# QuanjianSong/UniVST

Measured on AMD Instinct MI355X. Metric: stylized frames/sec, SD-v1.5 16x512x512 @50 DDIM steps, higher is better.
Workload: dtype f16; 1 GPU; sd15_unet_three_branch_pnp_transfer_16x512x512_50ddim; frames=16, branches=3, schedule_steps=53 (wrapping modulo 50), masks=moving disc, blended on steps 0..45, parallelism=single, weights=random-init SD-v1.5 architecture (859M + 201M temporal params), fp16

## Files before the change

### univst_amd/csrc/attention.hip

```cpp
#include <string.h>

#include "common.h"
#include "kernels.h"

namespace {

constexpr int KT = 64;
constexpr float DEFER = 8.f;

typedef __fp16 fh2 __attribute__((ext_vector_type(2)));

__device__ __forceinline__ float max3f(float a, float b, float c) {
    float r;
    asm("v_max3_f32 %0, %1, %2, %3" : "=v"(r) : "v"(a), "v"(b), "v"(c));
    return r;
}

__device__ __forceinline__ void attn_merge_coef(float m1, float l1, float m2, float l2, float& w1, float& w2) {
    const bool has1 = l1 > 0.f, has2 = l2 > 0.f;
    const float m = has1 ? (has2 ? fmaxf(m1, m2) : m1) : m2;
    const float a1 = has1 ? l1 * __builtin_amdgcn_exp2f(m1 - m) : 0.f;
    const float a2 = has2 ? __builtin_amdgcn_exp2f(m2 - m) : 0.f;
    const float den = a1 + l2 * a2;
    const float inv = den > 0.f ? 1.f / den : 0.f;
// ... 323 lines not shown
    for (int qb = 0; qb < QB; ++qb) {
        float l;
        if (ONES) {
            l = __shfl(o[DV16 - 1][qb][0], 32 + l15, 64);
        } else {
            l = lrun[qb];
            l += __shfl_xor(l, 16, 64);
            l += __shfl_xor(l, 32, 64);
        }
        float inv = 1.f / l, w1 = 0.f;
        const int qrow = qblk * 64 * QB + wave * 16 * QB + qb * 16 + l15;
        if (qrow >= p.Nq) continue;
        half_t* op = p.o + ((long)bf * p.Nq + qrow) * p.ldo + h * d;
        if constexpr (TP != 0) {
            const float m2 = CF ? mrun[qb] : mrun[qb] * c;
            const long srow = (((long)bf * p.heads + h) * p.Nq + qrow) * 2;
            if constexpr (TP == 1) {
                if (g == 0) *reinterpret_cast<float2*>(p.state_out + srow) = make_float2(m2, l);
            } else {
                const float2 st = *reinterpret_cast<const float2*>(p.state_in + srow);
                attn_merge_coef(st.x, st.y, m2, l, w1, inv);
            }
        }
#pragma unroll
        for (int dv = 0; dv < DV16; ++dv) {
            const int dc = dv * 16 + g * 4;
            if (dc < d) {
                h4 ov;
                if constexpr (TP == 2) {
                    const h4 o1 = *reinterpret_cast<const h4*>(op + dc);
#pragma unroll
                    for (int r = 0; r < 4; ++r) ov[r] = (half_t)fmaf((float)o1[r], w1, o[dv][qb][r] * inv);
                } else {
#pragma unroll
                    for (int r = 0; r < 4; ++r) ov[r] = (half_t)(o[dv][qb][r] * inv);
                }
                *reinterpret_cast<h4*>(op + dc) = ov;
            }
        }
    }
}

template <int DPAD, int DV16, int QB, bool CF = false, int TP = 0>
__global__ __launch_bounds__(256) void attn_kernel(AttnParams p) {
    attn_body<DPAD, DV16, QB, CF, TP>(p);
}
template <int DPAD, int DV16, int QB, bool CF = false, int TP = 0>
__global__ __launch_bounds__(256, 3) void attn_kernel_occ3(AttnParams p) {
    attn_body<DPAD, DV16, QB, CF, TP>(p);
}

__device__ __attribute__((aligned(256))) half_t uv_attn_zero_page[128];

template <int TAG = 0, int STG = 0, bool K16 = false, int TP = 0>
__global__ __launch_bounds__(256, 2) void attn_pp40_kernel(AttnParams p) {
    constexpr int NW = 4;
    constexpr int D = 40, DV16 = 3, QB = 4, NST = 3;
    constexpr int KSTR = lds_stride_bytes(64 * 2) / 2;
    constexpr int VSTR = lds_stride_bytes(48 * 2) / 2;
    constexpr int KPL = 512, VPL = 576;
    constexpr int KAREA = STG ? 8 * KPL : KT * KSTR;
    constexpr int TILE = STG ? 8 * KPL + 6 * VPL : KT * KSTR + KT * VSTR;
    __shared__ __attribute__((aligned(16))) half_t smem[NST * TILE];

    const int tid = threadIdx.x, lane = tid & 63, wave = tid >> 6;
    const int l15 = lane & 15, g = lane >> 4;
    const int nqb = (p.Nq + 64 * NW - 1) / (64 * NW);
    const int lid = xcd_remap(blockIdx.x, gridDim.x);
    const int qblk = lid % nqb;
    const int h = p.order ? lid / (nqb * p.BF) : (lid / nqb) % p.heads;
    const int bf = p.order ? (lid / nqb) % p.BF : lid / (nqb * p.heads);
    const h8 zero8 = {0, 0, 0, 0, 0, 0, 0, 0};

    const int ntile = (p.Nkv + KT - 1) / KT;
    const int nsrc_eff = p.src_cnt ? p.src_cnt[bf] : p.nsrc;
    const int T = nsrc_eff * ntile;
    if (TP && T == 0) {
        attn_empty_phase<64 * NW>(p, bf, h, qblk, D);
        return;
    }
    float lw_cur = p.src_logw ? p.src_logw[bf * p.nsrc] : 0.f;

    h8 qf[QB][2];
#pragma unroll
    for (int qb = 0; qb < QB; ++qb) {
        const int qrow = qblk * 64 * NW + wave * 16 * QB + qb * 16 + l15;
#pragma unroll
        for (int ks = 0; ks < 2; ++ks) {
            const int dc = ks * 32 + g * 8;
            h8 v = (qrow < p.Nq && dc < D) ? *reinterpret_cast<const h8*>(p.q + ((long)bf * p.Nq + qrow) * p.ldq + h * D + dc) : zero8;
            qf[qb][ks] = v;
        }
        if (!K16 && g == 1) qf[qb][1][2] = (half_t)lw_cur;
        if (K16) {
            h8 v = zero8;
            if (qrow < p.Nq && g < 2) {
                const h4 t = *reinterpret_cast<const h4*>(p.q + ((long)bf * p.Nq + qrow) * p.ldq + h * D + 32 + g * 4);
                v[0] = t[0]; v[1] = t[1]; v[2] = t[2]; v[3] = t[3];
            }
            if (g == 2) v[2] = (half_t)lw_cur;
            qf[qb][1] = v;
        }
    }
    auto set_shift = [&](int qb, float M) -> float {
        const float hi = floorf(M * 0.125f) * 8.f, lo = M - hi;
        const half_t hh = (half_t)(-hi), lh = (half_t)(-lo);
// ... 88 lines not shown
            const int pl = wave_u + NW * j;
            if ((j + 1) * NW <= 2 * DCH || pl < 2 * DCH) {
                const bool isv = pl >= DCH;
                const int c = isv ? pl - DCH : pl;
                const half_t* src = rok ? (isv ? p.v : p.k) + roff + c * 8 : zpage;
                const int dst = stage_half + (isv ? KAREA + c * VPL : c * KPL);
                glds16(src, __builtin_amdgcn_readfirstlane(smem_lds + 2u * (unsigned)dst));
            }
        }
        advance_ld();
    };
    {
        for (int i = tid * 8; i < NST * TILE; i += NW * 64 * 8) *reinterpret_cast<h8*>(&smem[i]) = zero8;
        __syncthreads();
        if (tid < KT) {
#pragma unroll
            for (int st = 0; st < NST; ++st) {
                if (STG) {
                    smem[st * TILE + KAREA + 5 * VPL + tid * 8] = (half_t)1.f;
                    smem[st * TILE + 5 * KPL + tid * 8] = (half_t)1.f;
                    smem[st * TILE + 5 * KPL + tid * 8 + 1] = (half_t)1.f;
                    smem[st * TILE + 5 * KPL + tid * 8 + 2] = (half_t)1.f;
                } else {
                    smem[st * TILE + KT * KSTR + tid * VSTR + D] = (half_t)1.f;
                    smem[st * TILE + tid * KSTR + D] = (half_t)1.f;
                    smem[st * TILE + tid * KSTR + D + 1] = (half_t)1.f;
                    smem[st * TILE + tid * KSTR + D + 2] = (half_t)1.f;
                }
            }
        }
        if (STG) __syncthreads();
    }

    const int kf_off = STG ? g * KPL + l15 * 8 : l15 * KSTR + g * 8;
    const int vf_off = STG ? KAREA + ((l15 & 3) >> 1) * VPL + (g * 4 + (l15 >> 2)) * 8 + (l15 & 1) * 4
                           : KT * KSTR + (g * 4 + (l15 >> 2)) * VSTR + (l15 & 3) * 4;
    auto kfrag_read = [&](const half_t* st, int hh, h8 (&kf)[2][2]) {
#pragma unroll
        for (int kb = 0; kb < 2; ++kb)
#pragma unroll
            for (int ks = 0; ks < 2; ++ks) {
                if (K16 && ks == 1) {
                    const int o16 = STG ? (4 + (g >> 1)) * KPL + l15 * 8 + (g & 1) * 4 + (hh * 32 + kb * 16) * 8
                                        : l15 * KSTR + 32 + g * 4 + (hh * 32 + kb * 16) * KSTR;
                    const h4 t = *reinterpret_cast<const h4*>(&st[o16]);
                    h8 v = zero8;
                    v[0] = t[0]; v[1] = t[1]; v[2] = t[2]; v[3] = t[3];
                    kf[kb][1] = v;
                } else {
                    kf[kb][ks] = *reinterpret_cast<const h8*>(&st[kf_off + (STG ? (hh * 32 + kb * 16) * 8 + ks * 4 * KPL : (hh * 32 + kb * 16) * KSTR + ks * 32)]);
                }
            }
    };
    auto vfrag_read = [&](const half_t* st, int hh, h8 (&vf)[DV16]) {
#pragma unroll
        for (int dv = 0; dv < DV16; ++dv) {
            const half_t* vp = &st[vf_off + (STG ? hh * 32 * 8 + dv * 2 * VPL : hh * 32 * VSTR + dv * 16)];
            fh4 lo = __builtin_amdgcn_ds_read_tr16_b64_v4f16((__attribute__((address_space(3))) fh4*)(vp));
            fh4 hi = __builtin_amdgcn_ds_read_tr16_b64_v4f16((__attribute__((address_space(3))) fh4*)(vp + 16 * (STG ? 8 : VSTR)));
            h8 a;
            a[0] = (half_t)lo[0]; a[1] = (half_t)lo[1]; a[2] = (half_t)lo[2]; a[3] = (half_t)lo[3];
            a[4] = (half_t)hi[0]; a[5] = (half_t)hi[1]; a[6] = (half_t)hi[2]; a[7] = (half_t)hi[3];
            vf[dv] = a;
        }
    };
    auto lo4 = [](const h8& v) { h4 r; r[0] = v[0]; r[1] = v[1]; r[2] = v[2]; r[3] = v[3]; return r; };
    auto qk_a = [&](const h8 (&kf)[2][2], f4 (&sc)[2][QB]) {
        const f4 z = {0.f, 0.f, 0.f, 0.f};
#pragma unroll
        for (int kb = 0; kb < 2; ++kb)
#pragma unroll
            for (int qb = 0; qb < QB; ++qb) sc[kb][qb] = __builtin_amdgcn_mfma_f32_16x16x16f16(lo4(kf[kb][1]), lo4(qf[qb][1]), z, 0, 0, 0);
    };
    auto qk_fence = [&](f4 (&sc)[2][QB]) {
        asm volatile("" : "+v"(qf[0][0]), "+v"(qf[1][0]), "+v"(qf[2][0]), "+v"(qf[3][0])
                     : "v"(sc[0][0]), "v"(sc[0][1]), "v"(sc[0][2]), "v"(sc[0][3]), "v"(sc[1][0]), "v"(sc[1][1]), "v"(sc[1][2]), "v"(sc[1][3]));
    };
    auto qk_b = [&](const h8 (&kf)[2][2], f4 (&sc)[2][QB]) {
#pragma unroll
        for (int kb = 0; kb < 2; ++kb)
#pragma unroll
            for (int qb = 0; qb < QB; ++qb) sc[kb][qb] = __builtin_amdgcn_mfma_f32_16x16x32_f16(kf[kb][0], qf[qb][0], sc[kb][qb], 0, 0, 0);
    };
    auto qk = [&](const h8 (&kf)[2][2], f4 (&sc)[2][QB]) {
        const f4 z = {0.f, 0.f, 0.f, 0.f};
        if (K16) {
            qk_a(kf, sc);
            qk_fence(sc);
            __builtin_amdgcn_sched_barrier(0);
            qk_b(kf, sc);
            return;
        }
#pragma unroll
        for (int kb = 0; kb < 2; ++kb)
#pragma unroll
            for (int qb = 0; qb < QB; ++qb) sc[kb][qb] = __builtin_amdgcn_mfma_f32_16x16x32_f16(kf[kb][0], qf[qb][0], z, 0, 0, 0);
#pragma unroll
        for (int kb = 0; kb < 2; ++kb)
#pragma unroll
            for (int qb = 0; qb < QB; ++qb) sc[kb][qb] = __builtin_amdgcn_mfma_f32_16x16x32_f16(kf[kb][1], qf[qb][1], sc[kb][qb], 0, 0, 0);
    };
    auto exp_part = [&](const f4 (&sc)[2][QB], h8 (&pb)[QB]) {
#pragma unroll
        for (int qb = 0; qb < QB; ++qb) {
            union { fh2 h[4]; h8 v; } u;
#pragma unroll
            for (int kb = 0; kb < 2; ++kb) {
                const float e0 = __builtin_amdgcn_exp2f(sc[kb][qb][0]), e1 = __builtin_amdgcn_exp2f(sc[kb][qb][1]);
                const float e2 = __builtin_amdgcn_exp2f(sc[kb][qb][2]), e3 = __builtin_amdgcn_exp2f(sc[kb][qb][3]);
                u.h[kb * 2] = __builtin_amdgcn_cvt_pkrtz(e0, e1);
                u.h[kb * 2 + 1] = __builtin_amdgcn_cvt_pkrtz(e2, e3);
            }
            pb[qb] = u.v;
        }
    };
    auto exp_half = [&](const f4 (&sc)[2][QB], h8 (&pb)[QB], int half) {
#pragma unroll
        for (int q2 = 0; q2 < 2; ++q2) {
            const int qb = half * 2 + q2;
            union { fh2 h[4]; h8 v; } u;
#pragma unroll
            for (int kb = 0; kb < 2; ++kb) {
                const float e0 = __builtin_amdgcn_exp2f(sc[kb][qb][0]), e1 = __builtin_amdgcn_exp2f(sc[kb][qb][1]);
                const float e2 = __builtin_amdgcn_exp2f(sc[kb][qb][2]), e3 = __builtin_amdgcn_exp2f(sc[kb][qb][3]);
                u.h[kb * 2] = __builtin_amdgcn_cvt_pkrtz(e0, e1);
                u.h[kb * 2 + 1] = __builtin_amdgcn_cvt_pkrtz(e2, e3);
            }
            pb[qb] = u.v;
        }
    };
    auto pv = [&](const h8 (&vf)[DV16], const h8 (&pb)[QB]) {
#pragma unroll
        for (int dv = 0; dv < DV16; ++dv)
#pragma unroll
            for (int qb = 0; qb < QB; ++qb) o[dv][qb] = __builtin_amdgcn_mfma_f32_16x16x32_f16(vf[dv], pb[qb], o[dv][qb], 0, 0, 0);
    };
    auto local_max = [&](const f4 (&sc)[2][QB], float (&mx)[QB]) {
#pragma unroll
        for (int qb = 0; qb < QB; ++qb) {
            float m = max3f(sc[0][qb][0], sc[0][qb][1], sc[0][qb][2]);
            m = max3f(m, sc[0][qb][3], sc[1][qb][0]);
            m = max3f(m, sc[1][qb][1], sc[1][qb][2]);
            mx[qb] = max3f(m, sc[1][qb][3], sc[1][qb][3]);
        }
    };
    auto mask_tail = [&](f4 (&sc)[2][QB], int key0) {
#pragma unroll
        for (int kb = 0; kb < 2; ++kb)
#pragma unroll
            for (int qb = 0; qb < QB; ++qb)
#pragma unroll
                for (int r = 0; r < 4; ++r)
                    if (key0 + kb * 16 + g * 4 + r >= p.Nkv) sc[kb][qb][r] = -INFINITY;
    };
    auto decide = [&](f4 (&sc)[2][QB], const float (&mx)[QB], bool first) {
        if (!first) {
            const float mall = fmaxf(max3f(mx[0], mx[1], mx[2]), mx[3]);
            if (__builtin_amdgcn_ballot_w64(mall > DEFER) == 0) return;
        }
#pragma unroll
        for (int qb = 0; qb < QB; ++qb) {
            if (__builtin_amdgcn_ballot_w64(first || mx[qb] > DEFER) != 0) {
                float m = mx[qb];
                const float o16 = __shfl_xor(m, 16, 64);
                m = max3f(m, o16, o16);
                const float o32 = __shfl_xor(m, 32, 64);
                m = max3f(m, o32, o32);
                float delta = floorf(m * 64.f + 0.5f) * (1.f / 64.f);
                if (!first) delta = fmaxf(delta, 0.f);
                const float mnew = set_shift(qb, mrun[qb] + delta);
                delta = mnew - mrun[qb];
                mrun[qb] = mnew;
                const float alpha = first ? 1.f : __builtin_amdgcn_exp2f(-delta);
#pragma unroll
                for (int kb = 0; kb < 2; ++kb) {
                    sc[kb][qb][0] -= delta; sc[kb][qb][1] -= delta; sc[kb][qb][2] -= delta; sc[kb][qb][3] -= delta;
                }
#pragma unroll
                for (int dv = 0; dv < DV16; ++dv) {
                    o[dv][qb][0] *= alpha; o[dv][qb][1] *= alpha; o[dv][qb][2] *= alpha; o[dv][qb][3] *= alpha;
                }
            }
        }
    };
    auto set_lw = [&](float lw) {
        if (g == (K16 ? 2 : 1)) {
#pragma unroll
            for (int qb = 0; qb < QB; ++qb) qf[qb][1][2] = (half_t)lw;
        }
    };
#define UV_PP_PHASE1()                                                            \
    _Pragma("unroll") for (int i_ = 0; i_ < 16; ++i_) {                           \
        __builtin_amdgcn_sched_group_barrier(0x008, 1, 0);                        \
        if (i_ < 6) __builtin_amdgcn_sched_group_barrier(0x100, 1, 0);            \
        __builtin_amdgcn_sched_group_barrier(0x400, 2, 0);                        \
        __builtin_amdgcn_sched_group_barrier(0x002, 1, 0);                        \
    }
 \
#define UV_PP_PHASE1H(DS)                                                         \
    _Pragma("unroll") for (int i_ = 0; i_ < 8; ++i_) {                            \
        __builtin_amdgcn_sched_group_barrier(0x008, 1, 0);                        \
        if ((DS) && i_ < 6) __builtin_amdgcn_sched_group_barrier(0x100, 1, 0);    \
        __builtin_amdgcn_sched_group_barrier(0x400, 2, 0);                        \
        __builtin_amdgcn_sched_group_barrier(0x002, 1, 0);                        \
    }
#define UV_PP_PHASE2()                                                            \
    _Pragma("unroll") for (int i_ = 0; i_ < 12; ++i_) {                           \
        __builtin_amdgcn_sched_group_barrier(0x008, 1, 0);                        \
        if (i_ < 4) __builtin_amdgcn_sched_group_barrier(0x100, 1, 0);            \
        __builtin_amdgcn_sched_group_barrier(0x002, 2, 0);                        \
    }

#define UV_PP_PIN4(a) asm volatile("" : "+v"(a[0]), "+v"(a[1]), "+v"(a[2]), "+v"(a[3]))
#define UV_PP_PIN2(a, i) asm volatile("" : "+v"(a[i]), "+v"(a[(i) + 1]))

    if (STG) {
        dma_tile(0);
        if (T > 1) dma_tile(TILE);
        asm volatile("s_waitcnt vmcnt(0)" ::: "memory");
    } else {
        load_tile();
        store_tile(smem);
        if (T > 1) {
            load_tile();
            store_tile(smem + TILE);
        }
    }
    __syncthreads();

    f4 scA[2][QB], scB[2][QB];
    h8 kf[2][2], vf[DV16], pb[QB];
    float mx[QB];
    int nx_s = 0, nx_t = (ntile > 1) ? 1 : 0;
    if (ntile == 1) nx_s = 1;
    float lw_nxt = (nx_s != 0 && nx_s < nsrc_eff && p.src_logw) ? p.src_logw[bf * p.nsrc + nx_s] : lw_cur;
    int t0_cur = 0, t0_nxt = nx_t * KT;
    half_t* b_cur = smem;
    half_t* b_nxt = smem + TILE;
    half_t* b_ld = smem + 2 * TILE;

    kfrag_read(b_cur, 0, kf);
    qk(kf, scA);
    if (t0_cur + KT > p.Nkv) mask_tail(scA, t0_cur);
    local_max(scA, mx);
    decide(scA, mx, true);
    kfrag_read(b_cur, 1, kf);

    for (int tt = 0; tt < T; ++tt) {
        const bool has_next = tt + 1 < T;
        if (tt + 2 < T) {
            if (STG) dma_tile((int)(b_ld - smem));
            else load_tile();
        }
        vfrag_read(b_cur, 0, vf);
        if (K16) {
            qk_a(kf, scB);
            exp_half(scA, pb, 0);
            UV_PP_PIN2(pb, 0);
            UV_PP_PHASE1H(1);
            qk_fence(scB);
            __builtin_amdgcn_sched_barrier(0);
            qk_b(kf, scB);
            exp_half(scA, pb, 1);
            UV_PP_PIN2(pb, 2);
            UV_PP_PHASE1H(0);
        } else {
            qk(kf, scB);
            exp_part(scA, pb);
            UV_PP_PIN4(pb);
            UV_PP_PHASE1();
        }
        __builtin_amdgcn_sched_barrier(0);
        if (t0_cur + KT > p.Nkv) mask_tail(scB, t0_cur + 32);
        kfrag_read(b_nxt, 0, kf);
        pv(vf, pb);
        local_max(scB, mx);
        UV_PP_PIN4(mx);
        UV_PP_PHASE2();
        __builtin_amdgcn_sched_barrier(0);
        decide(scB, mx, false);
        if (lw_nxt != lw_cur) set_lw(lw_nxt);
        vfrag_read(b_cur, 1, vf);
        if (K16) {
            qk_a(kf, scA);
            exp_half(scB, pb, 0);
            UV_PP_PIN2(pb, 0);
            UV_PP_PHASE1H(1);
            qk_fence(scA);
            __builtin_amdgcn_sched_barrier(0);
            qk_b(kf, scA);
            exp_half(scB, pb, 1);
            UV_PP_PIN2(pb, 2);
            UV_PP_PHASE1H(0);
        } else {
            qk(kf, scA);
            exp_part(scB, pb);
            UV_PP_PIN4(pb);
            UV_PP_PHASE1();
        }
        __builtin_amdgcn_sched_barrier(0);
        if (has_next && t0_nxt + KT > p.Nkv) mask_tail(scA, t0_nxt);
        kfrag_read(b_nxt, 1, kf);
        pv(vf, pb);
        local_max(scA, mx);
        UV_PP_PIN4(mx);
        UV_PP_PHASE2();
        __builtin_amdgcn_sched_barrier(0);
        if (has_next) decide(scA, mx, false);
        if (!STG && tt + 2 < T) store_tile(b_ld);
        if (STG) asm volatile("s_waitcnt vmcnt(0)" ::: "memory");
        __syncthreads();
        half_t* tb = b_cur; b_cur = b_nxt; b_nxt = b_ld; b_ld = tb;
        t0_cur = t0_nxt;
        lw_cur = lw_nxt;
        if (++nx_t == ntile) {
            nx_t = 0;
            if (++nx_s < nsrc_eff && p.src_logw) lw_nxt = p.src_logw[bf * p.nsrc + nx_s];
        }
        t0_nxt = nx_t * KT;
    }
#undef UV_PP_PHASE1
#undef UV_PP_PHASE1H
#undef UV_PP_PIN2
#undef UV_PP_PIN4
#undef UV_PP_PHASE2

#pragma unroll
    for (int qb = 0; qb < QB; ++qb) {
        const float l = __shfl(o[DV16 - 1][qb][0], 32 + l15, 64);
        float inv = 1.f / l, w1 = 0.f;
        const int qrow = qblk * 64 * NW + wave * 16 * QB + qb * 16 + l15;
        if (qrow >= p.Nq) continue;
        half_t* op = p.o + ((long)bf * p.Nq + qrow) * p.ldo + h * D;
        if constexpr (TP != 0) {
            const float m2 = mrun[qb];
            const long srow = (((long)bf * p.heads + h) * p.Nq + qrow) * 2;
            if constexpr (TP == 1) {
                if (g == 0) *reinterpret_cast<float2*>(p.state_out + srow) = make_float2(m2, l);
            } else {
                const float2 st = *reinterpret_cast<const float2*>(p.state_in + srow);
                attn_merge_coef(st.x, st.y, m2, l, w1, inv);
            }
        }
#pragma unroll
        for (int dv = 0; dv < DV16; ++dv) {
            const int dc = dv * 16 + g * 4;
            if (dc < D) {
                h4 ov;
                if constexpr (TP == 2) {
                    const h4 o1 = *reinterpret_cast<const h4*>(op + dc);
#pragma unroll
                    for (int r = 0; r < 4; ++r) ov[r] = (half_t)fmaf((float)o1[r], w1, o[dv][qb][r] * inv);
                } else {
#pragma unroll
                    for (int r = 0; r < 4; ++r) ov[r] = (half_t)(o[dv][qb][r] * inv);
                }
                *reinterpret_cast<h4*>(op + dc) = ov;
            }
        }
    }
}

template <int TAG = 0, int TP = 0>
__global__ __launch_bounds__(256, 2) void attn_pp64_kernel(AttnParams p) {
    constexpr int D = 64, QB = 4;
    constexpr int NW = 4, DV16 = D / 16, NST = 3;
    constexpr int KS = D / 32;
    constexpr int NDK = D / 8, NPV = D / 8;
    constexpr int RB = NW * 16 * QB;
    constexpr int KPL = 512, VPL = 576;
    constexpr int KAREA = NDK * KPL;
    constexpr int TILE = NDK * KPL + NPV * VPL;
    __shared__ __attribute__((aligned(16))) half_t smem[NST * TILE];

    const int tid = threadIdx.x, lane = tid & 63, wave = tid >> 6;
// ... 43 lines not shown
    const half_t* const zpage = uv_attn_zero_page;
    const unsigned smem_lds = (unsigned)(size_t)((__attribute__((address_space(3))) half_t*)smem);
    auto glds16 = [](const half_t* src, unsigned lds_byte) {
        unsigned keep;
        asm volatile("s_mov_b32 %0, m0\n\ts_mov_b32 m0, %2\n\ts_nop 0\n\tglobal_load_lds_dwordx4 %1, off\n\ts_mov_b32 m0, %0"
                     : "=&s"(keep) : "v"(src), "s"(lds_byte) : "memory");
    };
    const long xk_delta = p.kx ? (long)(p.kx - p.k) : 0, xv_delta = p.kx ? (long)(p.vx - p.v) : 0;
    int ld_s = 0, ld_t = 0;
    long ld_koff, ld_voff, ld_ld;
    int ld_nkv, ld_ntile;
    {
        const long off = (long)__builtin_amdgcn_readfirstlane(p.src_idx[bf * p.nsrc]) * p.Nkv * p.ldkv + h * D;
        ld_koff = off; ld_voff = off; ld_ld = p.ldkv; ld_nkv = p.Nkv; ld_ntile = ntile;
    }
    auto dma_tile = [&](int stage_half) {
        const int t0 = ld_t * KT;
        const bool rok = t0 + lane < ld_nkv;
        const long roff = (long)(t0 + lane) * ld_ld;
        const half_t* const ksrc = p.k + ld_koff + roff;
        const half_t* const vsrc = p.v + ld_voff + roff;
#pragma unroll
        for (int j = 0; j < (NDK + NPV + NW - 1) / NW; ++j) {
            const int pl = wave_u + NW * j;
            if ((j + 1) * NW <= NDK + NPV || pl < NDK + NPV) {
                const bool isv = pl >= NDK;
                const int c = isv ? pl - NDK : pl;
                const half_t* src = rok ? (isv ? vsrc : ksrc) + c * 8 : zpage;
                const int dst = stage_half + (isv ? KAREA + c * VPL : c * KPL);
                glds16(src, __builtin_amdgcn_readfirstlane(smem_lds + 2u * (unsigned)dst));
            }
        }
        if (++ld_t == ld_ntile) {
            ld_t = 0;
            ++ld_s;
            if (ld_s < nsrc_eff) {
                const long off = (long)__builtin_amdgcn_readfirstlane(p.src_idx[bf * p.nsrc + ld_s]) * p.Nkv * p.ldkv + h * D;
                ld_koff = off; ld_voff = off;
            } else if (ld_s < nseg) {
                const long off = (long)__builtin_amdgcn_readfirstlane(p.x_idx[bf]) * p.Nkv_x * p.ldkv_x + h * D;
                ld_koff = off + xk_delta; ld_voff = off + xv_delta; ld_ld = p.ldkv_x; ld_nkv = p.Nkv_x; ld_ntile = ntile_x;
            }
        }
    };

    const int kf_off = g * KPL + l15 * 8;
    const int vf_off = KAREA + ((l15 & 3) >> 1) * VPL + (g * 4 + (l15 >> 2)) * 8 + (l15 & 1) * 4;
    auto kfrag_read = [&](const half_t* st, int hh, h8 (&kf)[2][KS]) {
#pragma unroll
        for (int kb = 0; kb < 2; ++kb)
#pragma unroll
            for (int ks = 0; ks < KS; ++ks) kf[kb][ks] = *reinterpret_cast<const h8*>(&st[kf_off + (hh * 32 + kb * 16) * 8 + ks * 4 * KPL]);
    };
    auto vfrag_read = [&](const half_t* st, int hh, h8 (&vf)[DV16]) {
#pragma unroll
        for (int dv = 0; dv < DV16; ++dv) {
            const half_t* vp = &st[vf_off + hh * 32 * 8 + dv * 2 * VPL];
            fh4 lo = __builtin_amdgcn_ds_read_tr16_b64_v4f16((__attribute__((address_space(3))) fh4*)(vp));
            fh4 hi = __builtin_amdgcn_ds_read_tr16_b64_v4f16((__attribute__((address_space(3))) fh4*)(vp + 16 * 8));
            h8 a;
            a[0] = (half_t)lo[0]; a[1] = (half_t)lo[1]; a[2] = (half_t)lo[2]; a[3] = (half_t)lo[3];
            a[4] = (half_t)hi[0]; a[5] = (half_t)hi[1]; a[6] = (half_t)hi[2]; a[7] = (half_t)hi[3];
            vf[dv] = a;
        }
    };
    auto qk = [&](const h8 (&kf)[2][KS], f4 (&sc)[2][QB]) {
#pragma unroll
        for (int kb = 0; kb < 2; ++kb)
#pragma unroll
            for (int qb = 0; qb < QB; ++qb) sc[kb][qb] = __builtin_amdgcn_mfma_f32_16x16x32_f16(kf[kb][0], qf[qb][0], cfold[qb], 0, 0, 0);
#pragma unroll
        for (int ks = 1; ks < KS; ++ks)
#pragma unroll
            for (int kb = 0; kb < 2; ++kb)
#pragma unroll
                for (int qb = 0; qb < QB; ++qb) sc[kb][qb] = __builtin_amdgcn_mfma_f32_16x16x32_f16(kf[kb][ks], qf[qb][ks], sc[kb][qb], 0, 0, 0);
    };
    auto exp_part = [&](const f4 (&sc)[2][QB], h8 (&pb)[QB]) {
#pragma unroll
        for (int qb = 0; qb < QB; ++qb) {
            union { fh2 h[4]; h8 v; } u;
#pragma unroll
            for (int kb = 0; kb < 2; ++kb) {
                const float e0 = __builtin_amdgcn_exp2f(sc[kb][qb][0]), e1 = __builtin_amdgcn_exp2f(sc[kb][qb][1]);
                const float e2 = __builtin_amdgcn_exp2f(sc[kb][qb][2]), e3 = __builtin_amdgcn_exp2f(sc[kb][qb][3]);
                u.h[kb * 2] = __builtin_amdgcn_cvt_pkrtz(e0, e1);
                u.h[kb * 2 + 1] = __builtin_amdgcn_cvt_pkrtz(e2, e3);
            }
            pb[qb] = u.v;
        }
    };
    auto row_sums = [&](const h8 (&pb)[QB]) {
        const fh2 one2 = {(__fp16)1.f, (__fp16)1.f};
#pragma unroll
        for (int qb = 0; qb < QB; ++qb) {
            union { fh2 h[4]; h8 v; } u;
            u.v = pb[qb];
#pragma unroll
            for (int i = 0; i < 4; ++i) lsum[qb] = __builtin_amdgcn_fdot2(u.h[i], one2, lsum[qb], false);
        }
    };
    auto pv = [&](const h8 (&vf)[DV16], const h8 (&pb)[QB]) {
#pragma unroll
        for (int dv = 0; dv < DV16; ++dv)
#pragma unroll
            for (int qb = 0; qb < QB; ++qb) o[dv][qb] = __builtin_amdgcn_mfma_f32_16x16x32_f16(vf[dv], pb[qb], o[dv][qb], 0, 0, 0);
    };
    auto local_max = [&](const f4 (&sc)[2][QB], float (&mx)[QB]) {
#pragma unroll
        for (int qb = 0; qb < QB; ++qb) {
            float m = max3f(sc[0][qb][0], sc[0][qb][1], sc[0][qb][2]);
            m = max3f(m, sc[0][qb][3], sc[1][qb][0]);
            m = max3f(m, sc[1][qb][1], sc[1][qb][2]);
            mx[qb] = max3f(m, sc[1][qb][3], sc[1][qb][3]);
        }
    };
    auto mask_tail = [&](f4 (&sc)[2][QB], int key0, int nkv) {
#pragma unroll
        for (int kb = 0; kb < 2; ++kb)
#pragma unroll
            for (int qb = 0; qb < QB; ++qb)
#pragma unroll
                for (int r = 0; r < 4; ++r)
                    if (key0 + kb * 16 + g * 4 + r >= nkv) sc[kb][qb][r] = -INFINITY;
    };
    auto decide = [&](f4 (&sc)[2][QB], const float (&mx)[QB], float lw, bool first) {
        if (!first) {
            const float mall = fmaxf(max3f(mx[0], mx[1], mx[2]), mx[3]);
            if (__builtin_amdgcn_ballot_w64(mall > DEFER) == 0) return;
        }
#pragma unroll
        for (int qb = 0; qb < QB; ++qb) {
            if (__builtin_amdgcn_ballot_w64(first || mx[qb] > DEFER) != 0) {
                float m = mx[qb];
                const float o16 = __shfl_xor(m, 16, 64);
                m = max3f(m, o16, o16);
                const float o32 = __shfl_xor(m, 32, 64);
                m = max3f(m, o32, o32);
                float delta = floorf(m * 64.f + 0.5f) * (1.f / 64.f);
                if (!first) delta = fmaxf(delta, 0.f);
                if (!(delta > -3.0e38f)) delta = 0.f;
                mrun[qb] += delta;
                const float alpha = first ? 1.f : __builtin_amdgcn_exp2f(-delta);
                const float cnew = lw - mrun[qb];
                cfold[qb] = f4{cnew, cnew, cnew, cnew};
#pragma unroll
                for (int kb = 0; kb < 2; ++kb) {
                    sc[kb][qb][0] -= delta; sc[kb][qb][1] -= delta; sc[kb][qb][2] -= delta; sc[kb][qb][3] -= delta;
                }
                lsum[qb] *= alpha;
#pragma unroll
                for (int dv = 0; dv < DV16; ++dv) {
                    o[dv][qb][0] *= alpha; o[dv][qb][1] *= alpha; o[dv][qb][2] *= alpha; o[dv][qb][3] *= alpha;
                }
            }
        }
    };
    auto set_lw = [&](float lw) {
#pragma unroll
        for (int qb = 0; qb < QB; ++qb) {
            const float cnew = lw - mrun[qb];
            cfold[qb] = f4{cnew, cnew, cnew, cnew};
        }
    };
 \
 \
#define UV_P64_PHASE1()                                                           \
    _Pragma("unroll") for (int i_ = 0; i_ < 2 * KS * QB; ++i_) {                  \
        __builtin_amdgcn_sched_group_barrier(0x008, 1, 0);                        \
        if (i_ < 2 * DV16) __builtin_amdgcn_sched_group_barrier(0x100, 1, 0);     \
        if (i_ < 4 * QB) {                                                        \
            __builtin_amdgcn_sched_group_barrier(0x400, 2, 0);                    \
            __builtin_amdgcn_sched_group_barrier(0x002, 1, 0);                    \
        }                                                                         \
    }
#define UV_P64_PHASE2()                                                           \
    _Pragma("unroll") for (int i_ = 0; i_ < DV16 * QB; ++i_) {                    \
        __builtin_amdgcn_sched_group_barrier(0x008, 1, 0);                        \
        if (i_ < 2 * KS) __builtin_amdgcn_sched_group_barrier(0x100, 1, 0);       \
        if (i_ < 4 * QB) __builtin_amdgcn_sched_group_barrier(0x002, 2, 0);       \
    }
#define UV_P64_PIN4(a) asm volatile("" : "+v"(a[0]), "+v"(a[1]), "+v"(a[2]), "+v"(a[3]))

    dma_tile(0);
    if (T > 1) dma_tile(TILE);
    asm volatile("s_waitcnt vmcnt(0)" ::: "memory");
    __syncthreads();

    f4 scA[2][QB], scB[2][QB];
    h8 kf[2][KS], vf[DV16], pb[QB];
    float mx[QB];
    int cs_s = 0, cs_t = 0;
    int nkv_cur = seg_nkv(0), nkv_nxt = nkv_cur;
    int nx_s = 0, nx_t = 0;
    auto advance_nx = [&]() {
        if (++nx_t == seg_ntile(nx_s)) { nx_t = 0; ++nx_s; }
    };
    advance_nx();
    float lw_nxt = nx_s < nseg ? seg_lw(nx_s) : lw_cur;
    nkv_nxt = nx_s < nseg ? seg_nkv(nx_s) : nkv_cur;
    int t0_cur = 0, t0_nxt = nx_t * KT;
    half_t* b_cur = smem;
    half_t* b_nxt = smem + TILE;
    half_t* b_ld = smem + 2 * TILE;
    (void)cs_s; (void)cs_t;

    kfrag_read(b_cur, 0, kf);
    qk(kf, scA);
    if (t0_cur + KT > nkv_cur) mask_tail(scA, t0_cur, nkv_cur);
    local_max(scA, mx);
    decide(scA, mx, lw_cur, true);
    kfrag_read(b_cur, 1, kf);

    for (int tt = 0; tt < T; ++tt) {
        const bool has_next = tt + 1 < T;
        if (tt + 2 < T) dma_tile((int)(b_ld - smem));
        vfrag_read(b_cur, 0, vf);
        qk(kf, scB);
        exp_part(scA, pb);
        UV_P64_PIN4(pb);
        UV_P64_PHASE1();
        __builtin_amdgcn_sched_barrier(0);
        if (t0_cur + KT > nkv_cur) mask_tail(scB, t0_cur + 32, nkv_cur);
        kfrag_read(b_nxt, 0, kf);
        pv(vf, pb);
        local_max(scB, mx);
        row_sums(pb);
        UV_P64_PIN4(mx);
        UV_P64_PIN4(lsum);
        UV_P64_PHASE2();
        __builtin_amdgcn_sched_barrier(0);
        decide(scB, mx, lw_cur, false);
        if (lw_nxt != lw_cur) set_lw(lw_nxt);
        vfrag_read(b_cur, 1, vf);
        qk(kf, scA);
        exp_part(scB, pb);
        UV_P64_PIN4(pb);
        UV_P64_PHASE1();
        __builtin_amdgcn_sched_barrier(0);
        if (has_next && t0_nxt + KT > nkv_nxt) mask_tail(scA, t0_nxt, nkv_nxt);
        kfrag_read(b_nxt, 1, kf);
        pv(vf, pb);
        local_max(scA, mx);
        row_sums(pb);
        UV_P64_PIN4(mx);
        UV_P64_PIN4(lsum);
        UV_P64_PHASE2();
        __builtin_amdgcn_sched_barrier(0);
        if (has_next) decide(scA, mx, lw_nxt, false);
        asm volatile("s_waitcnt vmcnt(0)" ::: "memory");
        __syncthreads();
        half_t* tb = b_cur; b_cur = b_nxt; b_nxt = b_ld; b_ld = tb;
        t0_cur = t0_nxt;
        nkv_cur = nkv_nxt;
        lw_cur = lw_nxt;
        advance_nx();
        if (nx_s < nseg) {
            lw_nxt = seg_lw(nx_s);
            nkv_nxt = seg_nkv(nx_s);
        }
        t0_nxt = nx_t * KT;
    }
#undef UV_P64_PHASE1
#undef UV_P64_PHASE2
#undef UV_P64_PIN4

#pragma unroll
    for (int qb = 0; qb < QB; ++qb) {
        float l = lsum[qb];
        l += __shfl_xor(l, 16, 64);
        l += __shfl_xor(l, 32, 64);
        float inv = 1.f / l, w1 = 0.f;
        const int qrow = qblk * RB + wave * 16 * QB + qb * 16 + l15;
        if (qrow >= p.Nq) continue;
        half_t* op = p.o + ((long)bf * p.Nq + qrow) * p.ldo + h * D;
        if constexpr (TP != 0) {
            const long srow = (((long)bf * p.heads + h) * p.Nq + qrow) * 2;
            if constexpr (TP == 1) {
                if (g == 0) *reinterpret_cast<float2*>(p.state_out + srow) = make_float2(mrun[qb], l);
            } else {
                const float2 st = *reinterpret_cast<const float2*>(p.state_in + srow);
                attn_merge_coef(st.x, st.y, mrun[qb], l, w1, inv);
            }
        }
#pragma unroll
        for (int dv = 0; dv < DV16; ++dv) {
            h4 ov;
            if constexpr (TP == 2) {
                const h4 o1 = *reinterpret_cast<const h4*>(op + dv * 16 + g * 4);
#pragma unroll
                for (int r = 0; r < 4; ++r) ov[r] = (half_t)fmaf((float)o1[r], w1, o[dv][qb][r] * inv);
            } else {
#pragma unroll
                for (int r = 0; r < 4; ++r) ov[r] = (half_t)(o[dv][qb][r] * inv);
            }
            *reinterpret_cast<h4*>(op + dv * 16 + g * 4) = ov;
        }
    }
}

__global__ void tr16_probe_kernel(float* out) {
    __shared__ __attribute__((aligned(16))) half_t sm[64 * 16];
    for (int i = threadIdx.x; i < 64 * 16; i += 64) sm[i] = (half_t)(float)i;
    __syncthreads();
    const int lane = threadIdx.x, l15 = lane & 15, g = lane >> 4;
    const half_t* vp = &sm[(g * 4 + (l15 >> 2)) * 16 + (l15 & 3) * 4];
    fh4 v = __builtin_amdgcn_ds_read_tr16_b64_v4f16((__attribute__((address_space(3))) fh4*)(vp));
    for (int j = 0; j < 4; ++j) out[lane * 4 + j] = (float)v[j];
}

template <int D>
__global__ __launch_bounds__(256, 2) void attn_text_kernel(AttnParams p) {
    constexpr int KS = (D + 31) / 32, DV16 = (D + 15) / 16, NKF = 5, NKEY = NKF * 16, NIT = 8;
    constexpr int KSTR = KS * 32 + 16;
    constexpr int VSTR = DV16 * 16;
    constexpr int DCH = D / 8;
    __shared__ __attribute__((aligned(16))) half_t smem[NKEY * KSTR + NKEY * VSTR];
    half_t* const Ks = smem;
    half_t* const Vs = smem + NKEY * KSTR;

    const int tid = threadIdx.x, lane = tid & 63, wave = tid >> 6;
    const int l15 = lane & 15, g = lane >> 4;
    const int nchunk = (p.Nq + 128 * NIT - 1) / (128 * NIT);
    const int lid = xcd_remap(blockIdx.x, gridDim.x);
    const int chunk = lid % nchunk;
    const int h = (lid / nchunk) % p.heads;
// ... 267 lines not shown
```

Baseline: 5.944 frames/s.

## Cut VGPR pressure in pp40/p64 attention loops via skewed exp and scalar max

The per-block max array is replaced by a single scalar overall max, and per-block maxima are recomputed inside decide only when the rescale path runs. The exp/pack step is software-skewed so each cvt_pkrtz consumes the previous exp pair, and the schedule-group barriers are adjusted to match. V-fragment LDS addresses are now formed from one precomputed base with an explicit add, and l15 is pinned in the epilogue. Together these are meant to lower register pressure and address arithmetic in the hot loop, at the cost of redundant max work whenever a rescale happens.

```diff
diff --git a/univst_amd/csrc/attention.hip b/univst_amd/csrc/attention.hip
--- a/univst_amd/csrc/attention.hip
+++ b/univst_amd/csrc/attention.hip
@@ -399,6 +399,25 @@
 
 __device__ __attribute__((aligned(256))) half_t uv_attn_zero_page[128];
 
+template <int QB>
+__device__ __forceinline__ void pp_exp_skewed(const f4 (&sc)[2][QB], h8 (&pb)[QB], int q0, int nq) {
+    union { fh2 h[4]; h8 v; } u[QB];
+    float ea = 0.f, eb = 0.f;
+#pragma unroll
+    for (int i = 0; i < QB * 4; ++i) {
+        if (i < nq * 4) {
+            const int qb = q0 + i / 4, kb = (i / 2) % 2, hp = i % 2;
+            const float na = __builtin_amdgcn_exp2f(sc[kb][qb][hp * 2]), nb = __builtin_amdgcn_exp2f(sc[kb][qb][hp * 2 + 1]);
+            if (i > 0) u[(i - 1) / 4].h[(i - 1) % 4] = __builtin_amdgcn_cvt_pkrtz(ea, eb);
+            ea = na; eb = nb;
+        }
+    }
+    u[nq - 1].h[3] = __builtin_amdgcn_cvt_pkrtz(ea, eb);
+#pragma unroll
+    for (int q2 = 0; q2 < QB; ++q2)
+        if (q2 < nq) pb[q0 + q2] = u[q2].v;
+}
+
 template <int TAG = 0, int STG = 0, bool K16 = false, int TP = 0>
 __global__ __launch_bounds__(256, 2) void attn_pp40_kernel(AttnParams p) {
     constexpr int NW = 4;
@@ -593,12 +612,21 @@
                 }
             }
     };
-    auto vfrag_read = [&](const half_t* st, int hh, h8 (&vf)[DV16]) {
+    typedef __attribute__((address_space(3))) fh4* lds_fh4_ptr;
+    const unsigned vf_lds = smem_lds + 2u * (unsigned)vf_off;
+    auto vfrag_base = [&](const half_t* st) {
+        const unsigned sb = (unsigned)(reinterpret_cast<const char*>(st) - reinterpret_cast<const char*>(smem));
+        unsigned a;
+        asm volatile("v_add_u32 %0, %1, %2" : "=v"(a) : "s"(sb), "v"(vf_lds));
+        __builtin_amdgcn_sched_barrier(0);
+        return a;
+    };
+    auto vfrag_read = [&](unsigned base, int hh, h8 (&vf)[DV16]) {
 #pragma unroll
         for (int dv = 0; dv < DV16; ++dv) {
-            const half_t* vp = &st[vf_off + (STG ? hh * 32 * 8 + dv * 2 * VPL : hh * 32 * VSTR + dv * 16)];
-            fh4 lo = __builtin_amdgcn_ds_read_tr16_b64_v4f16((__attribute__((address_space(3))) fh4*)(vp));
-            fh4 hi = __builtin_amdgcn_ds_read_tr16_b64_v4f16((__attribute__((address_space(3))) fh4*)(vp + 16 * (STG ? 8 : VSTR)));
+            const unsigned vp = base + 2u * (unsigned)(STG ? hh * 32 * 8 + dv * 2 * VPL : hh * 32 * VSTR + dv * 16);
+            fh4 lo = __builtin_amdgcn_ds_read_tr16_b64_v4f16((lds_fh4_ptr)(size_t)(vp));
+            fh4 hi = __builtin_amdgcn_ds_read_tr16_b64_v4f16((lds_fh4_ptr)(size_t)(vp + 2u * 16 * (STG ? 8 : VSTR)));
             h8 a;
             a[0] = (half_t)lo[0]; a[1] = (half_t)lo[1]; a[2] = (half_t)lo[2]; a[3] = (half_t)lo[3];
             a[4] = (half_t)hi[0]; a[5] = (half_t)hi[1]; a[6] = (half_t)hi[2]; a[7] = (half_t)hi[3];
@@ -641,49 +669,32 @@
 #pragma unroll
             for (int qb = 0; qb < QB; ++qb) sc[kb][qb] = __builtin_amdgcn_mfma_f32_16x16x32_f16(kf[kb][1], qf[qb][1], sc[kb][qb], 0, 0, 0);
     };
-    auto exp_part = [&](const f4 (&sc)[2][QB], h8 (&pb)[QB]) {
+    auto exp_part = [&](const f4 (&sc)[2][QB], h8 (&pb)[QB]) { pp_exp_skewed<QB>(sc, pb, 0, QB); };
+    auto exp_half = [&](const f4 (&sc)[2][QB], h8 (&pb)[QB], int half) { pp_exp_skewed<QB>(sc, pb, half * 2, 2); };
+    auto pv = [&](const h8 (&vf)[DV16], const h8 (&pb)[QB]) {
+#pragma unroll
+        for (int dv = 0; dv < DV16; ++dv)
+#pragma unroll
+            for (int qb = 0; qb < QB; ++qb) o[dv][qb] = __builtin_amdgcn_mfma_f32_16x16x32_f16(vf[dv], pb[qb], o[dv][qb], 0, 0, 0);
+    };
+    auto local_max = [&](const f4 (&sc)[2][QB]) -> float {
+        float m[QB];
 #pragma unroll
         for (int qb = 0; qb < QB; ++qb) {
-            union { fh2 h[4]; h8 v; } u;
-#pragma unroll
-            for (int kb = 0; kb < 2; ++kb) {
-                const float e0 = __builtin_amdgcn_exp2f(sc[kb][qb][0]), e1 = __builtin_amdgcn_exp2f(sc[kb][qb][1]);
-                const float e2 = __builtin_amdgcn_exp2f(sc[kb][qb][2]), e3 = __builtin_amdgcn_exp2f(sc[kb][qb][3]);
-                u.h[kb * 2] = __builtin_amdgcn_cvt_pkrtz(e0, e1);
-                u.h[kb * 2 + 1] = __builtin_amdgcn_cvt_pkrtz(e2, e3);
-            }
-            pb[qb] = u.v;
-        }
-    };
-    auto exp_half = [&](const f4 (&sc)[2][QB], h8 (&pb)[QB], int half) {
-#pragma unroll
-        for (int q2 = 0; q2 < 2; ++q2) {
-            const int qb = half * 2 + q2;
-            union { fh2 h[4]; h8 v; } u;
-#pragma unroll
-            for (int kb = 0; kb < 2; ++kb) {
-                const float e0 = __builtin_amdgcn_exp2f(sc[kb][qb][0]), e1 = __builtin_amdgcn_exp2f(sc[kb][qb][1]);
-                const float e2 = __builtin_amdgcn_exp2f(sc[kb][qb][2]), e3 = __builtin_amdgcn_exp2f(sc[kb][qb][3]);
-                u.h[kb * 2] = __builtin_amdgcn_cvt_pkrtz(e0, e1);
-                u.h[kb * 2 + 1] = __builtin_amdgcn_cvt_pkrtz(e2, e3);
-            }
-            pb[qb] = u.v;
-        }
-    };
-    auto pv = [&](const h8 (&vf)[DV16], const h8 (&pb)[QB]) {
-#pragma unroll
-        for (int dv = 0; dv < DV16; ++dv)
-#pragma unroll
-            for (int qb = 0; qb < QB; ++qb) o[dv][qb] = __builtin_amdgcn_mfma_f32_16x16x32_f16(vf[dv], pb[qb], o[dv][qb], 0, 0, 0);
-    };
-    auto local_max = [&](const f4 (&sc)[2][QB], float (&mx)[QB]) {
-#pragma unroll
-        for (int qb = 0; qb < QB; ++qb) {
-            float m = max3f(sc[0][qb][0], sc[0][qb][1], sc[0][qb][2]);
-            m = max3f(m, sc[0][qb][3], sc[1][qb][0]);
-            m = max3f(m, sc[1][qb][1], sc[1][qb][2]);
-            mx[qb] = max3f(m, sc[1][qb][3], sc[1][qb][3]);
-        }
+            m[qb] = max3f(sc[0][qb][0], sc[0][qb][1], sc[0][qb][2]);
+            m[qb] = max3f(m[qb], sc[0][qb][3], sc[1][qb][0]);
+            m[qb] = max3f(m[qb], sc[1][qb][1], sc[1][qb][2]);
+        }
+        float a = max3f(m[0], sc[1][0][3], sc[1][1][3]);
+        a = max3f(a, m[1], sc[1][2][3]);
+        a = max3f(a, m[2], sc[1][3][3]);
+        return max3f(a, m[3], m[3]);
+    };
+    auto block_max = [&](const f4 (&sc)[2][QB], int qb) -> float {
+        float m = max3f(sc[0][qb][0], sc[0][qb][1], sc[0][qb][2]);
+        m = max3f(m, sc[0][qb][3], sc[1][qb][0]);
+        m = max3f(m, sc[1][qb][1], sc[1][qb][2]);
+        return max3f(m, sc[1][qb][3], sc[1][qb][3]);
     };
     auto mask_tail = [&](f4 (&sc)[2][QB], int key0) {
 #pragma unroll
@@ -694,15 +705,12 @@
                 for (int r = 0; r < 4; ++r)
                     if (key0 + kb * 16 + g * 4 + r >= p.Nkv) sc[kb][qb][r] = -INFINITY;
     };
-    auto decide = [&](f4 (&sc)[2][QB], const float (&mx)[QB], bool first) {
-        if (!first) {
-            const float mall = fmaxf(max3f(mx[0], mx[1], mx[2]), mx[3]);
-            if (__builtin_amdgcn_ballot_w64(mall > DEFER) == 0) return;
-        }
+    auto decide = [&](f4 (&sc)[2][QB], float mall, bool first) {
+        if (!first && __builtin_amdgcn_ballot_w64(mall > DEFER) == 0) return;
 #pragma unroll
         for (int qb = 0; qb < QB; ++qb) {
-            if (__builtin_amdgcn_ballot_w64(first || mx[qb] > DEFER) != 0) {
-                float m = mx[qb];
+            float m = block_max(sc, qb);
+            if (__builtin_amdgcn_ballot_w64(first || m > DEFER) != 0) {
                 const float o16 = __shfl_xor(m, 16, 64);
                 m = max3f(m, o16, o16);
                 const float o32 = __shfl_xor(m, 32, 64);
@@ -730,30 +738,34 @@
             for (int qb = 0; qb < QB; ++qb) qf[qb][1][2] = (half_t)lw;
         }
     };
+ \
 #define UV_PP_PHASE1()                                                            \
     _Pragma("unroll") for (int i_ = 0; i_ < 16; ++i_) {                           \
         __builtin_amdgcn_sched_group_barrier(0x008, 1, 0);                        \
         if (i_ < 6) __builtin_amdgcn_sched_group_barrier(0x100, 1, 0);            \
         __builtin_amdgcn_sched_group_barrier(0x400, 2, 0);                        \
-        __builtin_amdgcn_sched_group_barrier(0x002, 1, 0);                        \
-    }
+        if (i_ > 0) __builtin_amdgcn_sched_group_barrier(0x002, 1, 0);            \
+    }                                                                             \
+    __builtin_amdgcn_sched_group_barrier(0x002, 1, 0);
  \
 #define UV_PP_PHASE1H(DS)                                                         \
     _Pragma("unroll") for (int i_ = 0; i_ < 8; ++i_) {                            \
         __builtin_amdgcn_sched_group_barrier(0x008, 1, 0);                        \
         if ((DS) && i_ < 6) __builtin_amdgcn_sched_group_barrier(0x100, 1, 0);    \
         __builtin_amdgcn_sched_group_barrier(0x400, 2, 0);                        \
-        __builtin_amdgcn_sched_group_barrier(0x002, 1, 0);                        \
-    }
+        if (i_ > 0) __builtin_amdgcn_sched_group_barrier(0x002, 1, 0);            \
+    }                                                                             \
+    __builtin_amdgcn_sched_group_barrier(0x002, 1, 0);
 #define UV_PP_PHASE2()                                                            \
     _Pragma("unroll") for (int i_ = 0; i_ < 12; ++i_) {                           \
         __builtin_amdgcn_sched_group_barrier(0x008, 1, 0);                        \
         if (i_ < 4) __builtin_amdgcn_sched_group_barrier(0x100, 1, 0);            \
-        __builtin_amdgcn_sched_group_barrier(0x002, 2, 0);                        \
+        if (i_ < 8) __builtin_amdgcn_sched_group_barrier(0x002, 2, 0);            \
     }
 
 #define UV_PP_PIN4(a) asm volatile("" : "+v"(a[0]), "+v"(a[1]), "+v"(a[2]), "+v"(a[3]))
 #define UV_PP_PIN2(a, i) asm volatile("" : "+v"(a[i]), "+v"(a[(i) + 1]))
+#define UV_PP_PIN1(a) asm volatile("" : "+v"(a))
 
     if (STG) {
         dma_tile(0);
@@ -771,7 +783,7 @@
 
     f4 scA[2][QB], scB[2][QB];
     h8 kf[2][2], vf[DV16], pb[QB];
-    float mx[QB];
+    float mall;
     int nx_s = 0, nx_t = (ntile > 1) ? 1 : 0;
     if (ntile == 1) nx_s = 1;
     float lw_nxt = (nx_s != 0 && nx_s < nsrc_eff && p.src_logw) ? p.src_logw[bf * p.nsrc + nx_s] : lw_cur;
@@ -783,8 +795,8 @@
     kfrag_read(b_cur, 0, kf);
     qk(kf, scA);
     if (t0_cur + KT > p.Nkv) mask_tail(scA, t0_cur);
-    local_max(scA, mx);
-    decide(scA, mx, true);
+    mall = local_max(scA);
+    decide(scA, mall, true);
     kfrag_read(b_cur, 1, kf);
 
     for (int tt = 0; tt < T; ++tt) {
@@ -793,7 +805,7 @@
             if (STG) dma_tile((int)(b_ld - smem));
             else load_tile();
         }
-        vfrag_read(b_cur, 0, vf);
+        vfrag_read(vfrag_base(b_cur), 0, vf);
         if (K16) {
             qk_a(kf, scB);
             exp_half(scA, pb, 0);
@@ -815,13 +827,13 @@
         if (t0_cur + KT > p.Nkv) mask_tail(scB, t0_cur + 32);
         kfrag_read(b_nxt, 0, kf);
         pv(vf, pb);
-        local_max(scB, mx);
-        UV_PP_PIN4(mx);
+        mall = local_max(scB);
+        UV_PP_PIN1(mall);
         UV_PP_PHASE2();
         __builtin_amdgcn_sched_barrier(0);
-        decide(scB, mx, false);
+        decide(scB, mall, false);
         if (lw_nxt != lw_cur) set_lw(lw_nxt);
-        vfrag_read(b_cur, 1, vf);
+        vfrag_read(vfrag_base(b_cur), 1, vf);
         if (K16) {
             qk_a(kf, scA);
             exp_half(scB, pb, 0);
@@ -843,11 +855,11 @@
         if (has_next && t0_nxt + KT > p.Nkv) mask_tail(scA, t0_nxt);
         kfrag_read(b_nxt, 1, kf);
         pv(vf, pb);
-        local_max(scA, mx);
-        UV_PP_PIN4(mx);
+        mall = local_max(scA);
+        UV_PP_PIN1(mall);
         UV_PP_PHASE2();
         __builtin_amdgcn_sched_barrier(0);
-        if (has_next) decide(scA, mx, false);
+        if (has_next) decide(scA, mall, false);
         if (!STG && tt + 2 < T) store_tile(b_ld);
         if (STG) asm volatile("s_waitcnt vmcnt(0)" ::: "memory");
         __syncthreads();
@@ -862,6 +874,7 @@
     }
 #undef UV_PP_PHASE1
 #undef UV_PP_PHASE1H
+#undef UV_PP_PIN1
 #undef UV_PP_PIN2
 #undef UV_PP_PIN4
 #undef UV_PP_PHASE2
@@ -1011,12 +1024,21 @@
 #pragma unroll
             for (int ks = 0; ks < KS; ++ks) kf[kb][ks] = *reinterpret_cast<const h8*>(&st[kf_off + (hh * 32 + kb * 16) * 8 + ks * 4 * KPL]);
     };
-    auto vfrag_read = [&](const half_t* st, int hh, h8 (&vf)[DV16]) {
+    typedef __attribute__((address_space(3))) fh4* lds_fh4_ptr;
+    const unsigned vf_lds = smem_lds + 2u * (unsigned)vf_off;
+    auto vfrag_base = [&](const half_t* st) {
+        const unsigned sb = (unsigned)(reinterpret_cast<const char*>(st) - reinterpret_cast<const char*>(smem));
+        unsigned a;
+        asm volatile("v_add_u32 %0, %1, %2" : "=v"(a) : "s"(sb), "v"(vf_lds));
+        __builtin_amdgcn_sched_barrier(0);
+        return a;
+    };
+    auto vfrag_read = [&](unsigned base, int hh, h8 (&vf)[DV16]) {
 #pragma unroll
         for (int dv = 0; dv < DV16; ++dv) {
-            const half_t* vp = &st[vf_off + hh * 32 * 8 + dv * 2 * VPL];
-            fh4 lo = __builtin_amdgcn_ds_read_tr16_b64_v4f16((__attribute__((address_space(3))) fh4*)(vp));
-            fh4 hi = __builtin_amdgcn_ds_read_tr16_b64_v4f16((__attribute__((address_space(3))) fh4*)(vp + 16 * 8));
+            const unsigned vp = base + 2u * (unsigned)(hh * 32 * 8 + dv * 2 * VPL);
+            fh4 lo = __builtin_amdgcn_ds_read_tr16_b64_v4f16((lds_fh4_ptr)(size_t)(vp));
+            fh4 hi = __builtin_amdgcn_ds_read_tr16_b64_v4f16((lds_fh4_ptr)(size_t)(vp + 2u * 16 * 8));
             h8 a;
             a[0] = (half_t)lo[0]; a[1] = (half_t)lo[1]; a[2] = (half_t)lo[2]; a[3] = (half_t)lo[3];
             a[4] = (half_t)hi[0]; a[5] = (half_t)hi[1]; a[6] = (half_t)hi[2]; a[7] = (half_t)hi[3];
@@ -1035,20 +1057,7 @@
 #pragma unroll
                 for (int qb = 0; qb < QB; ++qb) sc[kb][qb] = __builtin_amdgcn_mfma_f32_16x16x32_f16(kf[kb][ks], qf[qb][ks], sc[kb][qb], 0, 0, 0);
     };
-    auto exp_part = [&](const f4 (&sc)[2][QB], h8 (&pb)[QB]) {
-#pragma unroll
-        for (int qb = 0; qb < QB; ++qb) {
-            union { fh2 h[4]; h8 v; } u;
-#pragma unroll
-            for (int kb = 0; kb < 2; ++kb) {
-                const float e0 = __builtin_amdgcn_exp2f(sc[kb][qb][0]), e1 = __builtin_amdgcn_exp2f(sc[kb][qb][1]);
-                const float e2 = __builtin_amdgcn_exp2f(sc[kb][qb][2]), e3 = __builtin_amdgcn_exp2f(sc[kb][qb][3]);
-                u.h[kb * 2] = __builtin_amdgcn_cvt_pkrtz(e0, e1);
-                u.h[kb * 2 + 1] = __builtin_amdgcn_cvt_pkrtz(e2, e3);
-            }
-            pb[qb] = u.v;
-        }
-    };
+    auto exp_part = [&](const f4 (&sc)[2][QB], h8 (&pb)[QB]) { pp_exp_skewed<QB>(sc, pb, 0, QB); };
     auto row_sums = [&](const h8 (&pb)[QB]) {
         const fh2 one2 = {(__fp16)1.f, (__fp16)1.f};
 #pragma unroll
@@ -1065,14 +1074,24 @@
 #pragma unroll
             for (int qb = 0; qb < QB; ++qb) o[dv][qb] = __builtin_amdgcn_mfma_f32_16x16x32_f16(vf[dv], pb[qb], o[dv][qb], 0, 0, 0);
     };
-    auto local_max = [&](const f4 (&sc)[2][QB], float (&mx)[QB]) {
+    auto local_max = [&](const f4 (&sc)[2][QB]) -> float {
+        float m[QB];
 #pragma unroll
         for (int qb = 0; qb < QB; ++qb) {
-            float m = max3f(sc[0][qb][0], sc[0][qb][1], sc[0][qb][2]);
-            m = max3f(m, sc[0][qb][3], sc[1][qb][0]);
-            m = max3f(m, sc[1][qb][1], sc[1][qb][2]);
-            mx[qb] = max3f(m, sc[1][qb][3], sc[1][qb][3]);
-        }
+            m[qb] = max3f(sc[0][qb][0], sc[0][qb][1], sc[0][qb][2]);
+            m[qb] = max3f(m[qb], sc[0][qb][3], sc[1][qb][0]);
+            m[qb] = max3f(m[qb], sc[1][qb][1], sc[1][qb][2]);
+        }
+        float a = max3f(m[0], sc[1][0][3], sc[1][1][3]);
+        a = max3f(a, m[1], sc[1][2][3]);
+        a = max3f(a, m[2], sc[1][3][3]);
+        return max3f(a, m[3], m[3]);
+    };
+    auto block_max = [&](const f4 (&sc)[2][QB], int qb) -> float {
+        float m = max3f(sc[0][qb][0], sc[0][qb][1], sc[0][qb][2]);
+        m = max3f(m, sc[0][qb][3], sc[1][qb][0]);
+        m = max3f(m, sc[1][qb][1], sc[1][qb][2]);
+        return max3f(m, sc[1][qb][3], sc[1][qb][3]);
     };
     auto mask_tail = [&](f4 (&sc)[2][QB], int key0, int nkv) {
 #pragma unroll
@@ -1083,15 +1102,12 @@
                 for (int r = 0; r < 4; ++r)
                     if (key0 + kb * 16 + g * 4 + r >= nkv) sc[kb][qb][r] = -INFINITY;
     };
-    auto decide = [&](f4 (&sc)[2][QB], const float (&mx)[QB], float lw, bool first) {
-        if (!first) {
-            const float mall = fmaxf(max3f(mx[0], mx[1], mx[2]), mx[3]);
-            if (__builtin_amdgcn_ballot_w64(mall > DEFER) == 0) return;
-        }
+    auto decide = [&](f4 (&sc)[2][QB], float mall, float lw, bool first) {
+        if (!first && __builtin_amdgcn_ballot_w64(mall > DEFER) == 0) return;
 #pragma unroll
         for (int qb = 0; qb < QB; ++qb) {
-            if (__builtin_amdgcn_ballot_w64(first || mx[qb] > DEFER) != 0) {
-                float m = mx[qb];
+            float m = block_max(sc, qb);
+            if (__builtin_amdgcn_ballot_w64(first || m > DEFER) != 0) {
                 const float o16 = __shfl_xor(m, 16, 64);
                 m = max3f(m, o16, o16);
                 const float o32 = __shfl_xor(m, 32, 64);
@@ -1128,11 +1144,10 @@
     _Pragma("unroll") for (int i_ = 0; i_ < 2 * KS * QB; ++i_) {                  \
         __builtin_amdgcn_sched_group_barrier(0x008, 1, 0);                        \
         if (i_ < 2 * DV16) __builtin_amdgcn_sched_group_barrier(0x100, 1, 0);     \
-        if (i_ < 4 * QB) {                                                        \
-            __builtin_amdgcn_sched_group_barrier(0x400, 2, 0);                    \
-            __builtin_amdgcn_sched_group_barrier(0x002, 1, 0);                    \
-        }                                                                         \
-    }
+        if (i_ < 4 * QB) __builtin_amdgcn_sched_group_barrier(0x400, 2, 0);       \
+        if (i_ > 0 && i_ <= 4 * QB) __builtin_amdgcn_sched_group_barrier(0x002, 1, 0); \
+    }                                                                             \
+    if (2 * KS * QB <= 4 * QB) __builtin_amdgcn_sched_group_barrier(0x002, 1, 0);
 #define UV_P64_PHASE2()                                                           \
     _Pragma("unroll") for (int i_ = 0; i_ < DV16 * QB; ++i_) {                    \
         __builtin_amdgcn_sched_group_barrier(0x008, 1, 0);                        \
@@ -1140,6 +1155,7 @@
         if (i_ < 4 * QB) __builtin_amdgcn_sched_group_barrier(0x002, 2, 0);       \
     }
 #define UV_P64_PIN4(a) asm volatile("" : "+v"(a[0]), "+v"(a[1]), "+v"(a[2]), "+v"(a[3]))
+#define UV_P64_PIN1(a) asm volatile("" : "+v"(a))
 
     dma_tile(0);
     if (T > 1) dma_tile(TILE);
@@ -1148,7 +1164,7 @@
 
     f4 scA[2][QB], scB[2][QB];
     h8 kf[2][KS], vf[DV16], pb[QB];
-    float mx[QB];
+    float mall;
     int cs_s = 0, cs_t = 0;
     int nkv_cur = seg_nkv(0), nkv_nxt = nkv_cur;
     int nx_s = 0, nx_t = 0;
@@ -1167,14 +1183,14 @@
     kfrag_read(b_cur, 0, kf);
     qk(kf, scA);
     if (t0_cur + KT > nkv_cur) mask_tail(scA, t0_cur, nkv_cur);
-    local_max(scA, mx);
-    decide(scA, mx, lw_cur, true);
+    mall = local_max(scA);
+    decide(scA, mall, lw_cur, true);
     kfrag_read(b_cur, 1, kf);
 
     for (int tt = 0; tt < T; ++tt) {
         const bool has_next = tt + 1 < T;
         if (tt + 2 < T) dma_tile((int)(b_ld - smem));
-        vfrag_read(b_cur, 0, vf);
+        vfrag_read(vfrag_base(b_cur), 0, vf);
         qk(kf, scB);
         exp_part(scA, pb);
         UV_P64_PIN4(pb);
@@ -1183,15 +1199,15 @@
         if (t0_cur + KT > nkv_cur) mask_tail(scB, t0_cur + 32, nkv_cur);
         kfrag_read(b_nxt, 0, kf);
         pv(vf, pb);
-        local_max(scB, mx);
+        mall = local_max(scB);
         row_sums(pb);
-        UV_P64_PIN4(mx);
+        UV_P64_PIN1(mall);
         UV_P64_PIN4(lsum);
         UV_P64_PHASE2();
         __builtin_amdgcn_sched_barrier(0);
-        decide(scB, mx, lw_cur, false);
+        decide(scB, mall, lw_cur, false);
         if (lw_nxt != lw_cur) set_lw(lw_nxt);
-        vfrag_read(b_cur, 1, vf);
+        vfrag_read(vfrag_base(b_cur), 1, vf);
         qk(kf, scA);
         exp_part(scB, pb);
         UV_P64_PIN4(pb);
@@ -1200,13 +1216,13 @@
         if (has_next && t0_nxt + KT > nkv_nxt) mask_tail(scA, t0_nxt, nkv_nxt);
         kfrag_read(b_nxt, 1, kf);
         pv(vf, pb);
-        local_max(scA, mx);
+        mall = local_max(scA);
         row_sums(pb);
-        UV_P64_PIN4(mx);
+        UV_P64_PIN1(mall);
         UV_P64_PIN4(lsum);
         UV_P64_PHASE2();
         __builtin_amdgcn_sched_barrier(0);
-        if (has_next) decide(scA, mx, lw_nxt, false);
+        if (has_next) decide(scA, mall, lw_nxt, false);
         asm volatile("s_waitcnt vmcnt(0)" ::: "memory");
         __syncthreads();
         half_t* tb = b_cur; b_cur = b_nxt; b_nxt = b_ld; b_ld = tb;
@@ -1222,15 +1238,18 @@
     }
 #undef UV_P64_PHASE1
 #undef UV_P64_PHASE2
+#undef UV_P64_PIN1
 #undef UV_P64_PIN4
 
+    int l15f = l15;
+    asm volatile("" : "+v"(l15f));
 #pragma unroll
     for (int qb = 0; qb < QB; ++qb) {
         float l = lsum[qb];
         l += __shfl_xor(l, 16, 64);
         l += __shfl_xor(l, 32, 64);
         float inv = 1.f / l, w1 = 0.f;
-        const int qrow = qblk * RB + wave * 16 * QB + qb * 16 + l15;
+        const int qrow = qblk * RB + wave * 16 * QB + qb * 16 + l15f;
         if (qrow >= p.Nq) continue;
         half_t* op = p.o + ((long)bf * p.Nq + qrow) * p.ldo + h * D;
         if constexpr (TP != 0) {
```

After: 5.991 frames/s, median of 6. No clear change (+0.8%).
